# TGALLOWAY1/ReinforcementLearning_Blokus

Hardware: AMD Instinct MI355X
Metric: MCTS random-rollout simulations/sec (20x20, 4p) at 1/2/4/8 MI355X (higher is better)
Workload: dtype u32; 1 GPU; config3: 256 concurrent games x 1024 random rollouts (arena semantics, frontier move order, Philox RNG) from GPU-generated 20-ply positions; games=256, rollouts_per_game=1024, root_plies=20, move_order=frontier, parallelism=dp1 (independent games per rank)

## Files before the change

### reinforcementlearning_blokus_amd/csrc/blokus_kernels.hip

```cpp
#include <hip/hip_runtime.h>

#include <math.h>
#include <stdint.h>
#include <stdio.h>
#include <stdlib.h>
#include <string.h>

#include <sched.h>

#include <mutex>
#include <thread>
#include <new>
#include <vector>

#include "../../include/blokus_hip.h"
#include "orient_table.h"

#define BK_TABLES_VERSION 1

#define BK_U_HOST 1
#define BK_U_MOVEGEN 2
#define BK_U_ROLLOUT 3
#define BK_U_ROLLOUT_FR 4
#define BK_U_ROLLOUT_FRH 5
// ... 2335 lines not shown
    d->used[q] = (uint16_t)sused;
    if (newsize - 1 == smask && sfill == sused) {
#pragma unroll 2
        for (uint32_t i = 0; i < newsize / 8; ++i) d4[i] = s4[i];
        return true;
    }
    const uint4 unused = make_uint4(0xFFFFFFFFu, 0xFFFFFFFFu, 0xFFFFFFFFu, 0xFFFFFFFFu);
#pragma unroll 2
    for (uint32_t i = 0; i < newsize / 8; ++i) d4[i] = unused;
    if (sused == 0) return true;
    const FsetRef t = fs_ref(d, q, htab);
#pragma unroll 1
    for (uint32_t i = 0; i <= smask / 8; ++i) {
        const uint4 v = s4[i];
        const uint32_t w[4] = {v.x, v.y, v.z, v.w};
#pragma unroll
        for (int j = 0; j < 8; ++j) {
            const int k = fs_key16(w, j);
            if (k >= 0) fs_insert_clean(t, newsize - 1, (int16_t)k);
        }
    }
    return true;
}

template <bool FR>
__device__ __forceinline__ void finish_game(const RolloutArgs& a, Game& g, const Slab& slab, uint32_t slot) {
    if (a.rng_io) {
        uint4 t[4];
#pragma unroll
        for (int q = 0; q < 4; ++q) t[q] = reinterpret_cast<const uint4*>(&slab.word(SLAB_RNG_BASE))[q];
#pragma unroll
        for (int q = 0; q < 4; ++q) reinterpret_cast<uint4*>(a.rng_io + (size_t)g.pid * 16)[q] = t[q];
    }
    if (a.out_states != nullptr) {
        store_state(a, g, slab, a.out_states + g.pid);
        if constexpr (FR) copy_fset_out(a.out_sets + g.pid, &a.fslab[slot].s, slab);
        if (a.out == nullptr) { g.pid = -1; return; }
    }
    bk_result r;
    memset(&r, 0, sizeof r);
    if (a.cfg.semantics != BK_SEM_ROLLOUT) {
        int best = -1000000;
        Quad sc{0, 0, 0, 0};
#pragma unroll 1
        for (int p = 0; p < 4; ++p) {
            const uint32_t* pl = slab.base + p * 20;
            const uint32_t r0 = pl[0], r19 = pl[19];
            int s = board_score(g, p);
            s += 5 * (int)((r0 & 1u) + ((r0 >> 19) & 1u) + (r19 & 1u) + ((r19 >> 19) & 1u));
            uint32_t centre = 0;
#pragma unroll
            for (int R = 8; R < 12; ++R) centre += __builtin_popcount(pl[R] & 0x00000F00u);
            s += 2 * (int)centre;
            sc.set(p, (uint32_t)s);
            best = s > best ? s : best;
        }
        uint8_t wm = 0;
#pragma unroll
        for (int p = 0; p < 4; ++p) {
            r.scores[p] = (int16_t)(int)sc.get(p);
            wm |= (uint8_t)(((int)sc.get(p) == best) << p);
        }
        r.winner_mask = wm;
        if (g.out == 0xFu || a.cfg.semantics != BK_SEM_ARENA) {
            r.passes = (uint16_t)(g.passes - g.since_move);
            r.turns = (uint16_t)(g.turns - g.since_move);
        } else {
            r.passes = (uint16_t)g.passes;
            r.turns = (uint16_t)g.turns;
            r.reserved[0] = (uint32_t)g.since_move;
            if (!(g.status & BK_STATUS_STOP)) g.status |= BK_STATUS_CAP;
        }
    } else {
        int best = -1000000;
#pragma unroll
        for (int p = 0; p < 4; ++p) {
            r.scores[p] = (int16_t)board_score_q(g, p);
            best = r.scores[p] > best ? r.scores[p] : best;
        }
        r.reward = board_score(g, g.root_player) - g.root_score;
        r.turns = (uint16_t)g.turns;
    }
    r.plies = (uint16_t)g.plies;
    r.draws = g.draws;
    r.status = (uint8_t)g.status;
    a.out[g.pid] = r;
    g.pid = -1;
}

template <bool FR, bool LIVE = false>
__device__ __forceinline__ void start_game(const RolloutArgs& a, Game& g, const Slab& slab, uint32_t slot, int32_t pid,
                                           const uint64_t* htab, uint4* lm = nullptr) {
    int32_t ri = a.root_index ? a.root_index[pid] : (pid % a.n_roots);
    bool bad_root = false;
    if (ri < 0 || ri >= a.n_roots) {
        atomicOr(&a.counter[2], BK_STICKY_ROOT);
        ri = 0;
        bad_root = true;
    }
    const bk_state* s = a.roots + ri;
    g.pid = pid;
    uint32_t occ[20];
#pragma unroll
    for (int R = 0; R < 20; ++R) occ[R] = 0;
#pragma unroll 1
    for (int p = 0; p < 4; ++p) {
        uint32_t cells = 0;
        uint64_t w[7];
#pragma unroll
        for (int k = 0; k < 7; ++k) w[k] = s->planes[p][k];
        uint32_t* dst = slab.base + p * 20;
#pragma unroll
        for (int R = 0; R < 20; ++R) {
            const uint32_t row = plane_row(w, R);
            dst[R] = row;
            occ[R] |= row;
            cells += __builtin_popcount(row);
        }
        g.cells.set(p, cells);
        g.used.set(p, s->used[p] & 0x1FFFFFu);
    }
#pragma unroll
    for (int R = 0; R < 20; ++R) slab.at(4, R) = occ[R];
    g.first = s->first_move & 0xFu;
    g.out = a.cfg.semantics != BK_SEM_ROLLOUT ? (s->out_mask & 0xFu) : 0u;
    g.move_count0 = s->move_count;
    g.cur = s->current_player & 3;
    g.plies = g.passes = g.turns = g.since_move = 0;
    g.root_player = g.cur;
    g.root_score = board_score(g, g.cur);
    g.draws = 0;
    g.pcount = 0;
    g.status = bad_root ? 4u : 0u;
    if constexpr (FR) {
        if (a.cfg.semantics == BK_SEM_ROLLOUT) {
            bk_fset* d = &a.fslab[slot].s;
            const bk_fset* src = a.root_sets + ri;
#pragma unroll 1
            for (int q = 0; q < 4; ++q) {
                if (!fs_copy_dev(d, q, src, htab)) g.status |= 2u;
                uint16_t* hq = slab_hdr(slab, q);
                hq[0] = d->mask[q];
                hq[1] = d->fill[q];
                hq[2] = d->used[q];
            }
            if constexpr (LIVE) init_live_masks(d, slab, lm);
        } else {
            uint4 nolm[4];
            copy_fset_in(&a.fslab[slot].s, slab, a.root_sets + ri, LIVE ? lm : nolm);
        }
    }
    g.hmask = a.seat_masks ? (a.seat_masks[pid] & 0xFu) : (uint32_t)a.cfg.heuristic_seats;
    g.smask = a.seat_masks ? ((a.seat_masks[pid] >> 4) & 0xFu) : 0u;
    g.turns0 = a.seat_masks ? s->reserved[0] : 0u;
    g.passes0 = a.seat_masks ? s->reserved[1] : 0u;
    g.cap = a.cfg.max_plies - (int32_t)g.turns0;
    g.forced = a.forced ? a.forced[pid] : -1;
    if (a.rng_io) {
        {
            uint4 t[4];
#pragma unroll
            for (int q = 0; q < 4; ++q) t[q] = reinterpret_cast<const uint4*>(a.rng_io + (size_t)pid * 16)[q];
#pragma unroll
            for (int q = 0; q < 4; ++q) reinterpret_cast<uint4*>(&slab.word(SLAB_RNG_BASE))[q] = t[q];
        }
    } else if (a.cfg.rng == BK_RNG_NUMPY_MT) {
        const int nstreams = a.cfg.seats_share_stream ? 1 : 4;
        for (int q = 0; q < nstreams; ++q) {
            const MtCursor m = mt_cursor_init(a.compat_seeds[(size_t)pid * 4 + q]);
            slab.word(SLAB_RNG_BASE + 4 * q + 0) = m.i;
            slab.word(SLAB_RNG_BASE + 4 * q + 1) = m.a;
            slab.word(SLAB_RNG_BASE + 4 * q + 2) = m.b;
            slab.word(SLAB_RNG_BASE + 4 * q + 3) = m.c;
        }
    }
}

__device__ __forceinline__ uint32_t draw_index(const RolloutArgs& a, Game& g, const Slab& slab, uint32_t slot,
                                               uint32_t n) {
    const uint32_t rng = n - 1u;
    if (rng == 0u) return 0u;
    const uint32_t mask = mask_for(rng);
    uint32_t v;
    if (a.cfg.rng == BK_RNG_NUMPY_MT) {
        const int q = a.cfg.seats_share_stream ? 0 : g.cur;
        uint32_t* base = slab.base + SLAB_RNG_BASE + 4 * q;
        MtCursor m;
        m.i = base[0]; m.a = base[1]; m.b = base[2]; m.c = base[3];
        bool ov = (g.status & 1u) != 0u;
        do {
            v = mt_cursor_next(m, ov) & mask;
            g.draws++;
        } while (v > rng && !ov);
        if (ov) g.status |= 1u;
        base[0] = m.i; base[1] = m.a; base[2] = m.b; base[3] = m.c;
        if (v > rng) v = 0;
    } else {
        do {
            v = philox_u32(g.pcount++, (uint32_t)g.pid + a.cfg.stream_base, a.cfg.seed) & mask;
            g.draws++;
        } while (v > rng);
    }
    return v;
}

__device__ __forceinline__ double draw_double(const RolloutArgs& a, Game& g, const Slab& slab) {
    uint32_t x0, x1;
    if (a.cfg.rng == BK_RNG_NUMPY_MT) {
        const int q = a.cfg.seats_share_stream ? 0 : g.cur;
        uint32_t* base = slab.base + SLAB_RNG_BASE + 4 * q;
        MtCursor m;
        m.i = base[0]; m.a = base[1]; m.b = base[2]; m.c = base[3];
        bool ov = (g.status & 1u) != 0u;
        x0 = mt_cursor_next(m, ov);
        x1 = mt_cursor_next(m, ov);
        if (ov) g.status |= 1u;
        base[0] = m.i; base[1] = m.a; base[2] = m.b; base[3] = m.c;
    } else {
        x0 = philox_u32(g.pcount++, (uint32_t)g.pid + a.cfg.stream_base, a.cfg.seed);
        x1 = philox_u32(g.pcount++, (uint32_t)g.pid + a.cfg.stream_base, a.cfg.seed);
    }
    g.draws += 2;
    return ((double)(x0 >> 5) * 67108864.0 + (double)(x1 >> 6)) * (1.0 / 9007199254740992.0);
}

__device__ __forceinline__ void stop_info(const RolloutArgs& a, const Game& g, const Planes& P, uint32_t* my, int lane,
                                       uint2* rows_lds, const bk_fset* fs, int fmask, int p, uint32_t avail,
                                       uint32_t total) {
#pragma clang fp contract(off)
    bk_stop_info si;
    si.n_legal = (int32_t)total;
    si.quick_index = 0;
    si.quick_reward = 0.0;
    if (a.quick_masks && ((a.quick_masks[g.pid] >> p) & 1u)) {
        (void)movegen_counts<true>(P, avail, my, lane);
        uint32_t k3[3] = {0u, 0u, 0u}, suf = 0u, cp = 0u;
        int n3 = 0;
#pragma unroll 1
        for (int gg = BK_NUM_ORIENTS - 1; gg >= 0 && n3 < 3; --gg) {
            cp += (my[(gg / 3) * WAVE + lane] >> (10 * (gg % 3))) & 0x3FFu;
            const uint32_t piece = kInfo[gg] & 0xFFu;
            if (gg == 0 || (kInfo[gg - 1] & 0xFFu) != piece) {
                const uint32_t s0 = total - suf - cp;
                for (uint32_t j = 0; j < cp && n3 < 3; ++j) k3[n3++] = s0 + j;
                suf += cp;
                cp = 0u;
            }
        }
        uint32_t kk3[3] = {0u, 0u, 0u};
        int g3[3] = {0, 0, 0};
#pragma unroll
        for (int i = 0; i < 3; ++i)
            if (i < n3) g3[i] = pick_orient(my, lane, k3[i], kk3[i]);
        double best = 0.0;
        int q = -1;
#pragma unroll
        for (int i = 0; i < 3; ++i) {
            if (i >= n3) continue;
#pragma unroll
            for (int R = 0; R < 20; ++R) rows_lds[R * WAVE] = make_uint2(P.b(R), P.c(R));
            int ar, ac;
            locate_move_frontier(g3[i], kk3[i], rows_lds, fs->key[p], fmask, ar, ac);
            const double d = __dadd_rn(fabs((double)ar - 9.5), fabs((double)ac - 9.5));
            if (q < 0 || d < best) { best = d; q = i; }
        }
        if (q >= 0) {
            si.quick_index = (int32_t)k3[q];
            const double size_term = (double)(kInfo[g3[q]] & 0xFFu) * 0.1, centre_term = (20.0 - best) * 0.05;
            si.quick_reward = size_term + centre_term;
        }
    }
    a.stop_out[g.pid] = si;
}

#define HBLOCK 128
#define HEUR_WORDS (84 * WAVE)
#define HEUR_PSUM 40

struct CaptureArgs {
    uint32_t ply_mask[4];
    uint32_t k;
    bk_state* states;
    bk_fset* sets;
    int32_t* turn;
};

__device__ __forceinline__ void capture_checkpoint(const RolloutArgs& a, const CaptureArgs& sn, const Game& g,
                                                   const Slab& slab, uint32_t slot) {
    const uint32_t c = g.move_count0 + (uint32_t)g.plies;
    if (c >= 128u) return;
    const uint32_t w = c >> 5, below = (1u << (c & 31u)) - 1u;
    const uint32_t m0 = sn.ply_mask[0], m1 = sn.ply_mask[1], m2 = sn.ply_mask[2], m3 = sn.ply_mask[3];
    const uint32_t mw = w == 0u ? m0 : (w == 1u ? m1 : (w == 2u ? m2 : m3));
    if (!((mw >> (c & 31u)) & 1u)) return;
    const uint32_t k = (uint32_t)__builtin_popcount(mw & below) + (w > 0u ? (uint32_t)__builtin_popcount(m0) : 0u) +
                       (w > 1u ? (uint32_t)__builtin_popcount(m1) : 0u) +
                       (w > 2u ? (uint32_t)__builtin_popcount(m2) : 0u);
    const size_t at = (size_t)g.pid * sn.k + k;
    store_state<false>(a, g, slab, sn.states + at);
    copy_fset_out(sn.sets + at, &a.fslab[slot].s, slab);
    sn.turn[at] = (int32_t)(g.turns0 + (uint32_t)g.turns);
}

template <bool FR, bool HEUR = false, bool SNAP = false>
__device__ __forceinline__ void rollout_body(const RolloutArgs& a, const CaptureArgs& sn = CaptureArgs{}) {
    constexpr int BLK = HEUR ? HBLOCK : BLOCK;
    constexpr int AREA = HEUR ? HEUR_WORDS : FR ? ROLL_WORDS_FR : ROLL_WORDS_PER_WAVE;
    constexpr int HS_WORDS = HEUR ? (int)(sizeof(HeurShared) + 7) / 4 : 0;
    constexpr bool HT_LDS = FR && HEUR;
    __shared__ __attribute__((aligned(16))) uint32_t lds[AREA * (BLK / WAVE) + (HT_LDS ? 2 * BK_CELLS : 0) + HS_WORDS];
    const int lane0 = threadIdx.x & (WAVE - 1), wv = __builtin_amdgcn_readfirstlane(threadIdx.x / WAVE);
    uint64_t* htab_lds = reinterpret_cast<uint64_t*>(lds + AREA * (BLK / WAVE));
    const uint64_t* htab = HT_LDS ? htab_lds : kCellHash;
    HeurShared* hs = reinterpret_cast<HeurShared*>(lds + AREA * (BLK / WAVE) + (HT_LDS ? 2 * BK_CELLS : 0));
    if constexpr (HT_LDS) {
        for (int i = threadIdx.x; i < BK_CELLS; i += BLK) htab_lds[i] = kCellHash[i];
    }
    if constexpr (HEUR) heur_shared_init(hs, threadIdx.x, BLK);
    if constexpr (HT_LDS || HEUR) __syncthreads();
    const uint32_t slot0 = blockIdx.x * BLK + threadIdx.x;
    uint32_t* const my = lds + wv * AREA;
    const bool arena = a.cfg.semantics != BK_SEM_ROLLOUT;
    const bool advance = a.cfg.semantics == BK_SEM_ADVANCE;
    const bool lm_in_slab = FR && !HEUR && a.cfg.rng == BK_RNG_PHILOX && a.rng_io == nullptr;

    Game g;
    g.pid = -1;
    bool done = false;
    uint32_t handed = 0;
    SECT_DECL
    for (uint32_t iter = 0;; ++iter) {
        uint32_t slot = slot0;
        int lane = lane0;
        asm volatile("" : "+v"(slot), "+v"(lane));
        const Slab slab{a.slab + (size_t)slot * SLAB_WORDS};
        uint2* const rows_lds = reinterpret_cast<uint2*>(my) + lane;
        double* const psum = reinterpret_cast<double*>(my + HEUR_PSUM * WAVE) + lane;
        SECT(0);
        for (int guard = 0; guard < 3 && !done; ++guard) {
            if (g.pid < 0) {
                int32_t next;
                if (a.handout == 0) {
                    next = (int32_t)atomicAdd(&a.counter[0], 1u);
                } else if (handed == 0u) {
                    next = (int32_t)slot;
                } else if (a.handout == 1) {
                    next = (int32_t)(slot + handed * a.nslots);
                } else {
                    next = slot < a.long_slots ? (int32_t)(a.nslots + atomicAdd(&a.counter[0], 1u)) : a.n_playouts;
                }
                ++handed;
                if (next >= a.n_playouts) { done = true; break; }
                if (HEUR && a.forced && a.forced[next] == BK_FORCE_SKIP) continue;
                if constexpr (FR && !HEUR)
                    start_game<true, true>(a, g, slab, slot, next, htab, live_masks(slab, &a.fslab[slot], lm_in_slab));
                else
                    start_game<FR>(a, g, slab, slot, next, htab);
            }
            if (arena) {
#pragma unroll 1
                for (int s = 0; s < 4 && ((g.out >> g.cur) & 1u) && g.out != 0xFu &&
                                (advance ? g.plies : g.turns) < g.cap; ++s) {
                    g.passes++; g.turns++; g.since_move++;
                    g.cur = (g.cur + 1) & 3;
                }
                if (g.out == 0xFu || (advance ? g.plies : g.turns) >= g.cap) {
                    finish_game<FR>(a, g, slab, slot);
                    continue;
                }
            } else if (g.plies >= g.cap) {
                finish_game<FR>(a, g, slab, slot);
                continue;
            }
            break;
        }
        if (__ballot(!done) == 0ull) break;
        if (iter > a.max_iters) {
            if (lane == 0) { atomicOr(&a.counter[1], 1u); atomicOr(&a.counter[2], BK_STICKY_GUARD); }
            break;
        }
        SECT(1);
        const bool idle = done || g.pid < 0;
        const int p = idle ? 0 : g.cur;
        Planes P;
        {
            uint32_t own[20], occ[20];
#pragma unroll
            for (int R = 0; R < 20; ++R) {
                own[R] = idle ? 0u : slab.at(p, R);
                occ[R] = idle ? 0u : slab.at(4, R);
            }
            derive_rows(own, occ, (g.first >> p) & 1u, p, P);
        }
        make_pairs(P);
        const uint32_t avail = idle ? 0u : (~g.used.get(p) & 0x1FFFFFu);
        uint32_t total;
        int gs = 0;
        uint32_t kk = 0;
        const bool forced = HEUR && !idle && g.forced >= 0;
        const bool heur = HEUR && !idle && !forced && ((g.hmask >> p) & 1u);
        double h_target = 0.0, h_R = 0.0, h_total = 0.0;
        uint32_t h_ok[20];
        bool h_unc = false;
        if constexpr (HEUR) {
            total = 0;
            if (__builtin_amdgcn_ballot_w64(!idle && !heur)) {
                const uint32_t t = movegen_counts<true>(P, heur ? 0u : avail, my, lane);
                if (!idle && !heur) {
                    total = t;
                    if (forced) {
                        gs = -1;
                        if ((g.forced & BK_FORCE_INDEX) && (uint32_t)(g.forced & ~BK_FORCE_INDEX) < t)
                            gs = pick_orient(my, lane, (uint32_t)(g.forced & ~BK_FORCE_INDEX), kk);
                    } else if (t > 0u && !((g.smask >> p) & 1u)) {
                        gs = pick_orient(my, lane, draw_index(a, g, slab, slot, t), kk);
                    }
                }
            }
            if (__builtin_amdgcn_ballot_w64(heur)) {
                const int edge_w = (g.move_count0 + g.plies) < 30 ? 6 : 3;
#pragma unroll
                for (int R = 0; R < 20; ++R) rows_lds[R * WAVE].x = P.b(R);
                const uint32_t t = heur_pass_a(P, heur ? avail : 0u, rows_lds, psum, hs, edge_w);
#pragma unroll
                for (int R = 0; R < 20; ++R) rows_lds[R * WAVE] = make_uint2(P.b(R), P.c(R));
                if (heur) {
                    total = t;
                    if (t > 0u) {
#pragma unroll 1
                        for (int q = 0; q < BK_PIECES; ++q) h_total += psum[q * WAVE];
                        h_target = draw_double(a, g, slab) * h_total;
                        gs = heur_pick_orient(psum, rows_lds, hs, edge_w, h_target, h_R, h_ok, h_unc);
                    }
                }
            }
        } else {
            total = movegen_counts<true>(P, avail, my, lane);
        }
        SECT(2);
        if (idle) continue;
        if (FR && total > 0u && ((g.smask >> p) & 1u) && !forced) {
            if constexpr (HEUR) {
                if (a.stop_out)
                    stop_info(a, g, P, my, lane, rows_lds, &a.fslab[slot].s, (int)*slab_hdr(slab, p), p, avail, total);
            }
            g.status |= BK_STATUS_STOP;
            finish_game<FR>(a, g, slab, slot);
            continue;
        }
        bool fmove = false;
        if constexpr (HEUR) {
            if (forced) {
                fmove = !(g.forced & BK_FORCE_INDEX);
                const int fg = g.forced / 400;
                const bool bad = total == 0u ||
                                 (fmove ? (fg >= BK_NUM_ORIENTS || !((avail >> ((kInfo[fg] & 0xFFu) - 1u)) & 1u))
                                        : gs < 0);
                if (bad) {
                    g.status |= BK_STATUS_BADFORCE;
                    finish_game<FR>(a, g, slab, slot);
                    continue;
                }
            }
        }
        if (total == 0u) {
            if (arena) {
                g.out |= 1u << p;
                g.passes++; g.turns++; g.since_move++;
                g.cur = (g.cur + 1) & 3;
            } else {
                finish_game<FR>(a, g, slab, slot);
            }
            continue;
        }
        if constexpr (!HEUR) {
            const uint32_t k = draw_index(a, g, slab, slot, total);
            gs = pick_orient(my, lane, k, kk);
        }
        OrientRow orow = orient_row(gs < 0 ? 0 : gs);
#pragma unroll
        for (int R = 0; R < 20; ++R) rows_lds[R * WAVE] = make_uint2(P.b(R), P.c(R));
        SECT(3);
        int ar, ac;
        if constexpr (FR) {
            const bk_fset* fs = &a.fslab[slot].s;
            const int fmask = (int)*slab_hdr(slab, p);
            if (fmove) {
                gs = g.forced / 400;
                ar = (g.forced % 400) / 20;
                ac = g.forced % 20;
                orow = orient_row(gs);
                locate_pass1(gs, rows_lds);
                if (!((rows_lds[ar * WAVE].y >> ac) & 1u)) ar = -1;
            } else if (heur && gs < 0) {
                ar = -1;
                ac = 0;
            } else if (heur) {
                const int edge_w = (g.move_count0 + g.plies) < 30 ? 6 : 3;
                heur_walk_frontier(gs, h_ok, rows_lds, fs->key[p], fmask, hs, edge_w, h_target, h_R, h_total,
                                   ar, ac, h_unc);
                if (h_unc) g.status |= BK_STATUS_UNCERT;
            } else {
                if constexpr (HEUR) {
                    locate_move_frontier(orow, kk, rows_lds, fs->key[p], fmask, ar, ac);
                } else {
                    const uint4 lmv = live_masks(slab, &a.fslab[slot], lm_in_slab)[p];
                    locate_move_frontier<2, true>(orow, kk, rows_lds, fs->key[p], fmask, ar, ac, lmv);
                }
            }
        } else {
            locate_move_lds(orow, kk, rows_lds, ar, ac);
        }
        if (HEUR && ar < 0) {
            g.status |= forced ? BK_STATUS_BADFORCE : BK_STATUS_UNCERT;
            finish_game<FR>(a, g, slab, slot);
            continue;
        }
        if constexpr (HEUR) g.forced = -1;
        SECT(4);
        const uint32_t info = orow.info;
        const int n = (int)((info >> 8) & 0xFFu);
        uint32_t m[5] = {0u, 0u, 0u, 0u, 0u};
#pragma unroll
        for (int q = 0; q < 5; ++q) {
            const uint32_t cell = orow.cell[q];
            const uint32_t bit = q < n ? (1u << (ac + (int)(cell & 0xFFu))) : 0u;
#pragma unroll
            for (int d = 0; d < 5; ++d) m[d] |= ((cell >> 8) == (uint32_t)d) ? bit : 0u;
        }
        {
            uint32_t ow[5], oc[5];
#pragma unroll
            for (int d = 0; d < 5; ++d) {
                ow[d] = m[d] ? slab.at(p, ar + d) : 0u;
                oc[d] = m[d] ? slab.at(4, ar + d) : 0u;
            }
#pragma unroll
            for (int d = 0; d < 5; ++d) {
                if (m[d]) {
                    slab.at(p, ar + d) = ow[d] | m[d];
                    slab.at(4, ar + d) = oc[d] | m[d];
                }
            }
        }
        SECT(5);
        if constexpr (FR) {
            int32_t cells[5];
#pragma unroll
            for (int q = 0; q < 5; ++q) {
                const uint32_t cell = q < n ? orow.cell[q] : orow.cell[0];
                cells[q] = (ar + (int)(cell >> 8)) * 20 + ac + (int)(cell & 0xFFu);
            }
            const uint64_t real = frontier_ops(rows_lds, slab, p, (g.first >> p) & 1u, orow, ar, ac, m);
            SECT(7);
            int16_t* lk = reinterpret_cast<int16_t*>(lds + wv * AREA) + 2 * lane;
#ifdef BK_SECTION_PROF
            auto mark = [&](int i) { SECT(i); };
#else
            NoMark mark;
#endif
            constexpr int STG = HEUR ? 128 : BK_FS_STAGE_FR;
            static_assert(STG / 2 + STG / 8 <= AREA / WAVE, "the resize scratch fits the area");
            bool placed;
            if constexpr (HEUR)
                placed = place_frontier<STG>(&a.fslab[slot], p, lk, htab, cells, real, mark, slab_hdr(slab, p),
                                             lk + 2 * WAVE * (STG / 2));
            else
                placed = place_frontier_onepass<STG>(&a.fslab[slot], p, lk, htab, cells, real, mark,
                                                     slab_hdr(slab, p), lk + 2 * WAVE * (STG / 2),
                                                     live_masks(slab, &a.fslab[slot], lm_in_slab) + p);
            if (!placed) g.status |= 2u;
        }
        SECT(6);
        g.cells.set(p, g.cells.get(p) + (uint32_t)n);
        g.used.set(p, g.used.get(p) | (1u << ((info & 0xFFu) - 1u)));
        g.first &= ~(1u << p);
        g.plies++; g.turns++; g.since_move = 0;
        g.cur = (g.cur + 1) & 3;
        if constexpr (SNAP) {
            if (!(g.status & 2u)) capture_checkpoint(a, sn, g, slab, slot);
        }
        if constexpr (FR) {
            if (g.status & 2u) finish_game<FR>(a, g, slab, slot);
        }
    }
    SECT_FLUSH;
}

#if BK_DEF(BK_U_ROLLOUT)
__global__ __launch_bounds__(BLOCK, ROLL_BLOCKS_PER_CU) void k_rollout(RolloutArgs a) { rollout_body<false>(a); }
#else
__global__ void k_rollout(RolloutArgs a);
#endif
#if BK_DEF(BK_U_ROLLOUT)
__global__ __launch_bounds__(BLOCK, ROLL_BLOCKS_PER_CU) void k_advance(RolloutArgs a) { rollout_body<false>(a); }
#else
__global__ void k_advance(RolloutArgs a);
#endif
#if BK_DEF(BK_U_ROLLOUT_FR)
__global__ __launch_bounds__(BLOCK, FR_BLOCKS_PER_CU) void k_rollout_fr(RolloutArgs a) { rollout_body<true>(a); }
#else
__global__ void k_rollout_fr(RolloutArgs a);
#endif
#if BK_DEF(BK_U_ROLLOUT_FRH)
__global__ __launch_bounds__(HBLOCK, 2) void k_rollout_fr_h(RolloutArgs a) { rollout_body<true, true>(a); }
#else
__global__ void k_rollout_fr_h(RolloutArgs a);
#endif
#if BK_DEF(BK_U_ROLLOUT_FRHS)
__global__ __launch_bounds__(HBLOCK, 2) void k_rollout_fr_hs(RolloutArgs a, CaptureArgs sn) {
    rollout_body<true, true, true>(a, sn);
}
#else
__global__ void k_rollout_fr_hs(RolloutArgs a, CaptureArgs sn);
#endif

#define FM_N 624
#define FM_M 397
#pragma clang fp contract(off)

__device__ __forceinline__ uint32_t mt_y(uint32_t a, uint32_t b) {
    const uint32_t y = (a & 0x80000000u) | (b & 0x7fffffffu);
    return (y >> 1) ^ ((y & 1u) ? 0x9908b0dfu : 0u);
}

__device__ __forceinline__ void twist_range(uint32_t* mt, int lo, int hi, int off, int lane) {
    for (int k0 = lo; k0 < hi; k0 += WAVE) {
        const int k = k0 + lane;
        uint32_t v = 0;
        if (k < hi) v = mt[k + off] ^ mt_y(mt[k], mt[k + 1]);
        __syncthreads();
        if (k < hi) mt[k] = v;
        __syncthreads();
    }
}

__device__ void py_twist(uint32_t* mt, int lane) {
    twist_range(mt, 0, FM_N - FM_M, FM_M, lane);
    twist_range(mt, FM_N - FM_M, 2 * (FM_N - FM_M), FM_M - FM_N, lane);
    twist_range(mt, 2 * (FM_N - FM_M), FM_N - 1, FM_M - FM_N, lane);
    if (lane == 0) mt[FM_N - 1] = mt[FM_M - 1] ^ mt_y(mt[FM_N - 1], mt[0]);
    __syncthreads();
}

__device__ __forceinline__ uint32_t py_next(uint32_t* mt, int& idx, int lane) {
    if (idx >= FM_N) { py_twist(mt, lane); idx = 0; }
    uint32_t y = mt[idx++];
    y ^= y >> 11; y ^= (y << 7) & 0x9d2c5680u; y ^= (y << 15) & 0xefc60000u; y ^= y >> 18;
    return y;
}

__device__ __forceinline__ double py_random(uint32_t* mt, int& idx, int lane) {
    const uint32_t a = py_next(mt, idx, lane) >> 5, b = py_next(mt, idx, lane) >> 6;
    return ((double)a * 67108864.0 + (double)b) * (1.0 / 9007199254740992.0);
}

template <int CTRL>
__device__ __forceinline__ void argmax_dpp_step(double& v, int& j) {
    const uint64_t b = (uint64_t)__double_as_longlong(v);
    const uint32_t lo = (uint32_t)__builtin_amdgcn_update_dpp((int)(uint32_t)b, (int)(uint32_t)b, CTRL, 0xF, 0xF, false);
    const uint32_t hi = (uint32_t)__builtin_amdgcn_update_dpp((int)(uint32_t)(b >> 32), (int)(uint32_t)(b >> 32), CTRL,
                                                              0xF, 0xF, false);
    const int oj = __builtin_amdgcn_update_dpp(j, j, CTRL, 0xF, 0xF, false);
    const double ov = __longlong_as_double((long long)(((uint64_t)hi << 32) | (uint64_t)lo));
    if (ov > v || (ov == v && oj < j)) { v = ov; j = oj; }
}
__device__ __forceinline__ void wave_argmax(double& v, int& j) {
    argmax_dpp_step<0xB1>(v, j);
    argmax_dpp_step<0x4E>(v, j);
    argmax_dpp_step<0x141>(v, j);
    argmax_dpp_step<0x140>(v, j);
    const uint64_t b = (uint64_t)__double_as_longlong(v);
    double bv = v;
    int bj = j;
#pragma unroll
    for (int r = 0; r < 4; ++r) {
        const uint32_t lo = (uint32_t)__builtin_amdgcn_readlane((int)(uint32_t)b, 16 * r);
        const uint32_t hi = (uint32_t)__builtin_amdgcn_readlane((int)(uint32_t)(b >> 32), 16 * r);
        const double ov = __longlong_as_double((long long)(((uint64_t)hi << 32) | (uint64_t)lo));
        const int oj = __builtin_amdgcn_readlane(j, 16 * r);
        if (r == 0 || ov > bv || (ov == bv && oj < bj)) { bv = ov; bj = oj; }
    }
    v = bv;
    j = bj;
}

struct PowFix {
    const int32_t* offsets;
    const int32_t* entries;
    int32_t rows;
};

__device__ __forceinline__ double fm_explore(double c, double L2, uint32_t v, uint32_t N, const PowFix& fx) {
    double s = sqrt(L2 / (double)v);
    if ((int32_t)N >= fx.rows) return c * s;
    const int32_t e0 = fx.offsets[N], e1 = fx.offsets[N + 1];
    for (int32_t e = e0; e < e1; ++e) {
        const int32_t w = fx.entries[e];
        if ((uint32_t)(w >> 1) == v) {
            const long long bits = __double_as_longlong(s);
            s = __longlong_as_double((w & 1) ? bits + 1 : bits - 1);
        }
    }
    return c * s;
}

__device__ __forceinline__ int fm_select(const uint32_t* visits, const double* total, int nch, int lane,
                                         double L2, uint32_t N, double c, const PowFix& fx) {
    double best = -1.0 / 0.0;
    int bj = 0x7fffffff;
    for (int j = lane; j < nch; j += WAVE) {
        const uint32_t vi = visits[j];
        const double u = total[j] / (double)vi + fm_explore(c, L2, vi, N, fx);
        if (u > best) { best = u; bj = j; }
    }
    wave_argmax(best, bj);
    return bj;
}

#define FM_LOG_LDS 1024
struct FastMctsArgs {
    int32_t n_games;
    const int32_t* offset;
    const int32_t* iterations;
    const double* base;
    uint32_t* mt_state;
    const double* log_table;
    int32_t log_len;
    PowFix fix;
    double c;
    bk_fastmcts_out* out;
    int32_t* visits_out;
    uint32_t* err;
};

#if BK_DEF(BK_U_FASTMCTS)
__global__ __launch_bounds__(WAVE) void k_fastmcts(FastMctsArgs a) {
    __shared__ uint32_t visits[BK_FASTMCTS_MAX_CHILDREN];
    __shared__ double total[BK_FASTMCTS_MAX_CHILDREN];
    __shared__ uint32_t mt[FM_N];
    __shared__ double ltab[FM_LOG_LDS];
    const int lane = threadIdx.x;
    const int game = blockIdx.x;
    if (game >= a.n_games) return;
    const int n = a.offset[game + 1] - a.offset[game];
    const int iters = a.iterations[game];
    const int nlt = iters + 1 < a.log_len ? (iters + 1 < FM_LOG_LDS ? iters + 1 : FM_LOG_LDS)
                                          : (a.log_len < FM_LOG_LDS ? a.log_len : FM_LOG_LDS);
    for (int k = lane; k < nlt; k += WAVE) ltab[k] = a.log_table[k];
    const double base = a.base[game];
    uint32_t* st = a.mt_state + (size_t)game * (FM_N + 1);
    for (int k = lane; k < FM_N; k += WAVE) mt[k] = st[k];
    int idx = (int)st[FM_N];
    for (int k = lane; k < n && k < BK_FASTMCTS_MAX_CHILDREN; k += WAVE) { visits[k] = 0; total[k] = 0.0; }
    __syncthreads();
    if (n > BK_FASTMCTS_MAX_CHILDREN || iters >= a.log_len) {
        if (lane == 0) { atomicOr(a.err, 1u); atomicOr(a.err + 1, BK_STICKY_FASTMCTS); }
        return;
    }
    int nch = 0;
    uint32_t root_visits = 0;
    int it = 0;
    if (n <= 2 * WAVE) {
        __shared__ double fm_rew[FM_N / 2];
        const bool draw = base == base;
        uint32_t v0 = 0u, v1 = 0u;
        double t0 = 0.0, t1 = 0.0;
        int rptr = 0, ravail = 0, ridx = idx;
        for (; it < iters; ++it) {
            int sel;
            if (nch < n) {
                sel = nch++;
            } else {
                const double lg = (int)root_visits < nlt ? ltab[root_visits] : a.log_table[root_visits];
                const double L2 = 2.0 * lg;
                double best = -1.0 / 0.0;
                int bj = 0x7fffffff;
                if (lane < nch) { best = t0 / (double)v0 + fm_explore(a.c, L2, v0, root_visits, a.fix); bj = lane; }
                if (lane + WAVE < nch) {
                    const double u = t1 / (double)v1 + fm_explore(a.c, L2, v1, root_visits, a.fix);
                    if (u > best) { best = u; bj = lane + WAVE; }
                }
                wave_argmax(best, bj);
                sel = bj;
            }
            double reward = 0.0;
            if (draw) {
                if (rptr == ravail) {
                    idx = ridx;
                    if (idx >= FM_N) { py_twist(mt, lane); idx = 0; }
                    const int m = (FM_N - idx) / 2;
                    __syncthreads();
                    if (m == 0) {
                        const double r = py_random(mt, idx, lane);
                        if (lane == 0) fm_rew[0] = base + r * 0.1;
                        ravail = 1;
                    } else {
                        for (int l = lane; l < m; l += WAVE) {
                            uint32_t x = mt[idx + 2 * l], y = mt[idx + 2 * l + 1];
                            x ^= x >> 11; x ^= (x << 7) & 0x9d2c5680u; x ^= (x << 15) & 0xefc60000u; x ^= x >> 18;
                            y ^= y >> 11; y ^= (y << 7) & 0x9d2c5680u; y ^= (y << 15) & 0xefc60000u; y ^= y >> 18;
                            const double r = ((double)(x >> 5) * 67108864.0 + (double)(y >> 6)) *
                                             (1.0 / 9007199254740992.0);
                            fm_rew[l] = base + r * 0.1;
                        }
                        ravail = m;
                        idx += 2 * m;
                    }
                    ridx = idx;
                    rptr = 0;
                    __syncthreads();
                }
                reward = fm_rew[rptr++];
            }
            if (lane == (sel & (WAVE - 1))) {
                if (sel < WAVE) { v0 += 1u; t0 += reward; }
                else { v1 += 1u; t1 += reward; }
            }
            root_visits += 1u;
        }
        if (draw) idx = ridx - 2 * (ravail - rptr);
        if (lane < n) { visits[lane] = v0; total[lane] = t0; }
        if (lane + WAVE < n) { visits[lane + WAVE] = v1; total[lane + WAVE] = t1; }
        __syncthreads();
    } else {
        for (; it < iters; ++it) {
            int sel;
            if (nch < n) {
                sel = nch++;
            } else {
                const double lg = (int)root_visits < nlt ? ltab[root_visits] : a.log_table[root_visits];
                sel = fm_select(visits, total, nch, lane, 2.0 * lg, root_visits, a.c, a.fix);
            }
            const double reward = (base == base) ? base + py_random(mt, idx, lane) * 0.1 : 0.0;
            if (lane == 0) {
                visits[sel] += 1u;
                total[sel] += reward;
            }
            __syncthreads();
            root_visits += 1u;
        }
    }
    if (a.visits_out) {
        int32_t* vo = a.visits_out + a.offset[game];
        for (int k = lane; k < n; k += WAVE) vo[k] = (n - 1 - k < nch) ? (int32_t)visits[n - 1 - k] : 0;
    }
    for (int k = lane; k < FM_N; k += WAVE) st[k] = mt[k];
    if (lane == 0) st[FM_N] = (uint32_t)idx;
    bk_fastmcts_out* o = a.out + game;
    if (lane == 0) { o->iterations = it; o->n_children = nch; }
    {
        double bv = -1.0;
        int bj = 0x7fffffff;
        for (int j = lane; j < nch; j += WAVE)
            if ((double)visits[j] > bv) { bv = (double)visits[j]; bj = j; }
        wave_argmax(bv, bj);
        if (lane == 0) o->best_index = nch > 0 ? n - 1 - bj : 0;
    }
    int ntop = 0;
    for (int t = 0; t < BK_FASTMCTS_TOP && t < nch; ++t) {
        double bv = -1.0;
        int bj = 0x7fffffff;
        for (int j = lane; j < nch; j += WAVE)
            if (!(visits[j] & 0x80000000u) && (double)visits[j] > bv) { bv = (double)visits[j]; bj = j; }
        wave_argmax(bv, bj);
        if (lane == 0) {
            const uint32_t v = visits[bj];
            o->top_index[t] = n - 1 - bj;
            o->top_visits[t] = (int32_t)v;
            o->top_q[t] = total[bj] / (double)v;
            visits[bj] = v | 0x80000000u;
        }
        __syncthreads();
        ++ntop;
    }
    if (lane == 0) o->n_top = ntop;
}
#else
__global__ void k_fastmcts(FastMctsArgs a);
#endif

#if BK_DEF(BK_U_FASTMCTS)
__global__ __launch_bounds__(WAVE) void k_fastmcts_select(const uint32_t* visits, const double* totals, int n,
                                                          uint32_t N, double L2, double c, PowFix fx, int32_t* out) {
    const int j = fm_select(visits, totals, n, threadIdx.x, L2, N, c, fx);
    if (threadIdx.x == 0) *out = j;
}
#else
__global__ void k_fastmcts_select(const uint32_t* visits, const double* totals, int n, uint32_t N, double L2, double c,
                                  PowFix fx, int32_t* out);
#endif

#define MC_FATAL(st) ((st) & ~BK_MCTS_EUNCERT)
#define MC_SELECT 0
#define MC_EXPAND 1
#define MC_ROLLOUT 2
#define MC_PATH (BK_MCTS_MAX_DEPTH + 1)
#define MC_ZOB 2088
#define MC_TREE_BATCH WAVE

struct McLane {
    FsLane A;
    bk_fset root;
// ... 4400 lines not shown
```

Measured before the change: 48.50 million sims/s.

## Let idle lanes probe other seats' moves for active games to skip passes early

New measurement: 49.14 million sims/s (median of 6 runs). 1.01x the previous value.

```diff
diff --git a/reinforcementlearning_blokus_amd/csrc/blokus_kernels.hip b/reinforcementlearning_blokus_amd/csrc/blokus_kernels.hip
--- a/reinforcementlearning_blokus_amd/csrc/blokus_kernels.hip
+++ b/reinforcementlearning_blokus_amd/csrc/blokus_kernels.hip
@@ -2661,8 +2661,62 @@
     sn.turn[at] = (int32_t)(g.turns0 + (uint32_t)g.turns);
 }
 
-template <bool FR, bool HEUR = false, bool SNAP = false>
+#define HELP_POST 31
+#define HELP_USED 32
+#define HELP_PAIR 36
+#define HELP_FOUND 37
+static_assert(CNT_DWORDS <= HELP_POST && HELP_FOUND < ROLL_WORDS_FR / WAVE, "the hand-over dwords are free");
+
+__device__ __forceinline__ void wave_lds_sync() {
+    __builtin_amdgcn_fence(__ATOMIC_RELEASE, "wavefront");
+    __builtin_amdgcn_wave_barrier();
+    __builtin_amdgcn_fence(__ATOMIC_ACQUIRE, "wavefront");
+}
+
+__device__ __forceinline__ bool help_assign(uint32_t* my, int lane, uint64_t clients, const Game& g,
+                                            uint32_t& client_lane, int& q, uint32_t& first, uint32_t& avail) {
+    const bool idle = !((clients >> lane) & 1ull);
+    const uint32_t below = (uint32_t)__popcll(clients & ((1ull << lane) - 1ull));
+    const uint32_t rank = idle ? (uint32_t)lane - below : below;
+    my[HELP_FOUND * WAVE + lane] = 0u;
+    my[HELP_PAIR * WAVE + lane] = 0u;
+    if (!idle) {
+        my[HELP_POST * WAVE + rank] = (uint32_t)lane | ((uint32_t)g.cur << 8) |
+                                      (((g.out | (g.status >> 8)) & 0xFu) << 12) | ((g.first & 0xFu) << 16);
+        my[(HELP_USED + 0) * WAVE + rank] = g.used.v0;
+        my[(HELP_USED + 1) * WAVE + rank] = g.used.v1;
+        my[(HELP_USED + 2) * WAVE + rank] = g.used.v2;
+        my[(HELP_USED + 3) * WAVE + rank] = g.used.v3;
+    }
+    wave_lds_sync();
+    const uint32_t c = rank / 3u, k = rank - 3u * c;
+    if (!idle || c >= (uint32_t)__popcll(clients)) return false;
+    const uint32_t post = my[HELP_POST * WAVE + c];
+    const uint32_t cur = (post >> 8) & 3u, open = ~(post >> 12) & 0xFu;
+    uint32_t r = ((open | (open << 4)) >> cur) & 0xEu;
+    if (k >= 1u) r &= r - 1u;
+    if (k >= 2u) r &= r - 1u;
+    if (r == 0u) return false;
+    q = (int)((cur + (uint32_t)__builtin_ctz(r)) & 3u);
+    client_lane = post & (WAVE - 1);
+    first = (post >> (16 + q)) & 1u;
+    avail = ~my[(HELP_USED + q) * WAVE + c] & 0x1FFFFFu;
+    my[HELP_PAIR * WAVE + lane] = client_lane | ((uint32_t)q << 6) | 0x100u;
+    return true;
+}
+
+__device__ __forceinline__ void help_report(uint32_t* my, int lane, bool idle, uint32_t total, Game& g) {
+    if (idle) {
+        const uint32_t pair = my[HELP_PAIR * WAVE + lane];
+        if (pair != 0u && total == 0u) atomicOr(&my[HELP_FOUND * WAVE + (pair & (WAVE - 1))], 1u << ((pair >> 6) & 3u));
+    }
+    wave_lds_sync();
+    if (!idle) g.status |= my[HELP_FOUND * WAVE + lane] << 8;
+}
+
+template <bool FR, bool HEUR = false, bool SNAP = false, bool HELP = false>
 __device__ __forceinline__ void rollout_body(const RolloutArgs& a, const CaptureArgs& sn = CaptureArgs{}) {
+    static_assert(!HELP || (FR && !HEUR && !SNAP), "the look-ahead is k_rollout_fr's");
     constexpr int BLK = HEUR ? HBLOCK : BLOCK;
     constexpr int AREA = HEUR ? HEUR_WORDS : FR ? ROLL_WORDS_FR : ROLL_WORDS_PER_WAVE;
     constexpr int HS_WORDS = HEUR ? (int)(sizeof(HeurShared) + 7) / 4 : 0;
@@ -2682,6 +2736,7 @@
     const bool arena = a.cfg.semantics != BK_SEM_ROLLOUT;
     const bool advance = a.cfg.semantics == BK_SEM_ADVANCE;
     const bool lm_in_slab = FR && !HEUR && a.cfg.rng == BK_RNG_PHILOX && a.rng_io == nullptr;
+    const bool help = HELP && a.cfg.semantics == BK_SEM_ARENA;
 
     Game g;
     g.pid = -1;
@@ -2718,8 +2773,9 @@
             }
             if (arena) {
 #pragma unroll 1
-                for (int s = 0; s < 4 && ((g.out >> g.cur) & 1u) && g.out != 0xFu &&
+                for (int s = 0; s < 4 && (((HELP ? g.out | (g.status >> 8) : g.out) >> g.cur) & 1u) && g.out != 0xFu &&
                                 (advance ? g.plies : g.turns) < g.cap; ++s) {
+                    if constexpr (HELP) g.out |= 1u << g.cur;
                     g.passes++; g.turns++; g.since_move++;
                     g.cur = (g.cur + 1) & 3;
                 }
@@ -2738,21 +2794,31 @@
             if (lane == 0) { atomicOr(&a.counter[1], 1u); atomicOr(&a.counter[2], BK_STICKY_GUARD); }
             break;
         }
+        const bool idle = done || g.pid < 0;
+        bool helping = false;
+        uint32_t h_lane = 0, h_first = 0, h_avail = 0;
+        int h_q = 0;
+        if constexpr (HELP) {
+            const uint64_t clients = __ballot(!idle);
+            if (help && clients != ~0ull)
+                helping = help_assign(my, lane, clients, g, h_lane, h_q, h_first, h_avail);
+        }
         SECT(1);
-        const bool idle = done || g.pid < 0;
-        const int p = idle ? 0 : g.cur;
+        const int p = HELP && helping ? h_q : idle ? 0 : g.cur;
         Planes P;
         {
+            const Slab src{HELP && helping ? a.slab + (size_t)(slot - (uint32_t)lane + h_lane) * SLAB_WORDS : slab.base};
+            const bool blank = HELP ? idle && !helping : idle;
             uint32_t own[20], occ[20];
 #pragma unroll
             for (int R = 0; R < 20; ++R) {
-                own[R] = idle ? 0u : slab.at(p, R);
-                occ[R] = idle ? 0u : slab.at(4, R);
-            }
-            derive_rows(own, occ, (g.first >> p) & 1u, p, P);
+                own[R] = blank ? 0u : src.at(p, R);
+                occ[R] = blank ? 0u : src.at(4, R);
+            }
+            derive_rows(own, occ, HELP && helping ? h_first : (g.first >> p) & 1u, p, P);
         }
         make_pairs(P);
-        const uint32_t avail = idle ? 0u : (~g.used.get(p) & 0x1FFFFFu);
+        const uint32_t avail = HELP && helping ? h_avail : idle ? 0u : (~g.used.get(p) & 0x1FFFFFu);
         uint32_t total;
         int gs = 0;
         uint32_t kk = 0;
@@ -2797,6 +2863,9 @@
             total = movegen_counts<true>(P, avail, my, lane);
         }
         SECT(2);
+        if constexpr (HELP) {
+            if (help && __ballot(idle) != 0ull) help_report(my, lane, idle, total, g);
+        }
         if (idle) continue;
         if (FR && total > 0u && ((g.smask >> p) & 1u) && !forced) {
             if constexpr (HEUR) {
@@ -2957,7 +3026,9 @@
 __global__ void k_advance(RolloutArgs a);
 #endif
 #if BK_DEF(BK_U_ROLLOUT_FR)
-__global__ __launch_bounds__(BLOCK, FR_BLOCKS_PER_CU) void k_rollout_fr(RolloutArgs a) { rollout_body<true>(a); }
+__global__ __launch_bounds__(BLOCK, FR_BLOCKS_PER_CU) void k_rollout_fr(RolloutArgs a) {
+    rollout_body<true, false, false, true>(a);
+}
 #else
 __global__ void k_rollout_fr(RolloutArgs a);
 #endif
```
